# apache/orc

Hardware: AMD Instinct MI355X
Metric: decoded GB/s + Mvalues/s device-resident, RLEv2 int64 column at 1/2/4/8 GPU (higher is better)
Workload: dtype int64; 1 GPU; configs[1]: single int64 RLEv2-direct column, 10^8 rows, uncompressed stream resident in HBM, 1 MI355X per stripe; rows_per_gpu=100000000, encoding=RLEv2 DIRECT, W=64 (aligned), 512-value runs, signed (zigzag), stream_bytes=800390626, row_index_stride=10000, parallelism=stripe-sharded x1, kernel=rlev2_tiled_kernel, variant=0

## Files before the change

include/orcg_reader.h:

```cpp
#ifndef ORCG_READER_H
#define ORCG_READER_H

#include "orcg.h"

#ifdef __cplusplus
extern "C" {
#endif

enum {
  ORCG_TYPE_BOOLEAN = 0, ORCG_TYPE_BYTE = 1, ORCG_TYPE_SHORT = 2, ORCG_TYPE_INT = 3, ORCG_TYPE_LONG = 4,
  ORCG_TYPE_FLOAT = 5, ORCG_TYPE_DOUBLE = 6, ORCG_TYPE_STRING = 7, ORCG_TYPE_BINARY = 8,
  ORCG_TYPE_TIMESTAMP = 9, ORCG_TYPE_LIST = 10, ORCG_TYPE_MAP = 11, ORCG_TYPE_STRUCT = 12,
  ORCG_TYPE_UNION = 13, ORCG_TYPE_DECIMAL = 14, ORCG_TYPE_DATE = 15, ORCG_TYPE_VARCHAR = 16,
  ORCG_TYPE_CHAR = 17, ORCG_TYPE_TIMESTAMP_INSTANT = 18
};
enum { ORCG_COMPRESSION_NONE = 0, ORCG_COMPRESSION_ZLIB = 1, ORCG_COMPRESSION_SNAPPY = 2,
       ORCG_COMPRESSION_LZO = 3, ORCG_COMPRESSION_LZ4 = 4, ORCG_COMPRESSION_ZSTD = 5 };

typedef struct orcg_reader orcg_reader;

typedef struct {
  uint32_t kind;
  uint32_t num_subtypes;
  uint32_t maximum_length;
// ... 93 lines not shown
int orcg_reader_last_timings(const orcg_reader* r, double* out5);
int orcg_reader_last_stream_stats(const orcg_reader* r, uint64_t* out2);
typedef struct orcg_reader_metrics {
  uint64_t reader_call;
  uint64_t reader_inclusive_latency_us;
  uint64_t decompression_call;
  uint64_t decompression_latency_us;
  uint64_t decoding_call;
  uint64_t decoding_latency_us;
  uint64_t byte_decoding_call;
  uint64_t byte_decoding_latency_us;
  uint64_t io_count;
  uint64_t io_blocking_latency_us;
  uint64_t selected_row_group_count;
  uint64_t evaluated_row_group_count;
  uint64_t read_range_cache_hits;
  uint64_t read_range_cache_misses;
} orcg_reader_metrics;
int orcg_reader_get_metrics(orcg_reader* r, orcg_reader_metrics* out);
int orcg_reader_reset_metrics(orcg_reader* r);
int orcg_reader_set_metrics_timing(orcg_reader* r, int on);
uint64_t orcg_reader_last_batched_streams(const orcg_reader* r);
uint64_t orcg_reader_last_stage_bytes(const orcg_reader* r);
int orcg_reader_set_stream_batching(orcg_reader* r, int on);

#ifdef __cplusplus
}
#endif
#endif
```

orc_amd/_lib.py:

```python
import ctypes
import os

HERE = os.path.dirname(os.path.abspath(__file__))
LIB_PATH = os.path.join(HERE, os.environ.get("ORCG_LIB", "liborcgpu.so"))

ORCG_OK = 0
ORCG_PARSE_ERROR = 1
ORCG_INVALID_ARGUMENT = 2
ORCG_DEVICE_ERROR = 3
ORCG_OUT_OF_MEMORY = 4


class OrcError(RuntimeError):
    status = None


class ParseError(OrcError):

    status = ORCG_PARSE_ERROR


class InvalidArgument(OrcError):

    status = ORCG_INVALID_ARGUMENT
# ... 145 lines not shown
    ("orcg_reader_stripe_column", [vp, u64, u32, ctypes.POINTER(ColumnView)], i32),
    ("orcg_reader_copy_to_host", [vp, vp, vp, u64], i32),
    ("orcg_reader_last_timings", [vp, ctypes.POINTER(ctypes.c_double)], i32),
    ("orcg_reader_last_stream_stats", [vp, ctypes.POINTER(u64)], i32),
    ("orcg_reader_get_metrics", [vp, ctypes.POINTER(u64)], i32),
    ("orcg_reader_reset_metrics", [vp], i32),
    ("orcg_reader_set_metrics_timing", [vp, i32], i32),
    ("orcg_reader_content_length", [vp], u64),
    ("orcg_reader_software_version", [vp], cp),
    ("orcg_reader_num_metadata", [vp], u32),
    ("orcg_reader_metadata_key", [vp, u32], cp),
    ("orcg_reader_metadata_value", [vp, u32, ctypes.POINTER(u64)], vp),
    ("orcg_reader_set_lazy_dictionary", [vp, i32], i32),
    ("orcg_reader_set_hive11_decimal", [vp, i32, i32], i32),
    ("orcg_reader_hive11_scale", [vp], i32),
    ("orcg_reader_set_read_type", [vp, cp], i32),
    ("orcg_reader_set_throw_on_schema_evolution_overflow", [vp, i32], i32),
    ("orcg_reader_read_type", [vp, u32, ctypes.POINTER(TypeInfo)], i32),
    ("orcg_reader_set_zone_rules", [vp, cp, cp, u64], i32),
    ("orcg_reader_set_timezone_name", [vp, cp], i32),
    ("orcg_reader_set_local_timezone", [vp, cp], i32),
    ("orcg_reader_last_batched_streams", [vp], u64),
    ("orcg_reader_last_stage_bytes", [vp], u64),
    ("orcg_reader_set_stream_batching", [vp, i32], i32),
    ("orcg_reader_is_selected", [vp, u32], i32),
    ("orcg_row_reader_create", [vp, ctypes.POINTER(RowReaderOptions), ctypes.POINTER(vp)], i32),
    ("orcg_row_reader_destroy", [vp], None),
    ("orcg_row_reader_next", [vp, u64, ctypes.POINTER(u64)], i32),
    ("orcg_row_reader_is_selected", [vp, u32], i32),
    ("orcg_row_reader_stripe", [vp], u64),
    ("orcg_row_reader_row_number", [vp], u64),
    ("orcg_host_alloc", [u64], vp),
    ("orcg_host_free", [vp], None),
    ("orcg_row_reader_last_error", [vp], cp),
    ("orcg_row_reader_timings", [vp, ctypes.POINTER(ctypes.c_double)], i32),
    ("orcg_row_reader_seek_to_row", [vp, u64], i32),
    ("orcg_row_reader_column", [vp, u32, ctypes.POINTER(ColumnView), ctypes.POINTER(u64), ctypes.POINTER(u64)],
     i32),
]

i64 = ctypes.c_int64
SIGNATURES += [
    ("orcg_arrow_validity_device", [vp, vp, u64, vp, u64, ctypes.POINTER(u64)], i32),
    ("orcg_arrow_fixed_device", [vp, i32, vp, vp, u64, vp, u64], i32),
    ("orcg_arrow_offsets_device", [vp, vp, vp, vp, u64, vp, u64], i32),
    ("orcg_arrow_dict_strings_device", [vp, i32, vp, vp, u64, vp, u64, vp, u64, vp, u64, vp, u64,
# ... 71 lines not shown
```

orc_amd/build.py:

```python
import os
import subprocess
import sys

HERE = os.path.dirname(os.path.abspath(__file__))
CSRC = os.path.join(HERE, "csrc")
PROF = os.environ.get("ORCG_PHASE_PROF", "") == "1"
AB = os.environ.get("ORCG_AB", "") == "1"
OUT = os.path.join(HERE, "liborcgpu_prof.so" if PROF else ("liborcgpu_ab.so" if AB else "liborcgpu.so"))
OBJ = os.path.join(HERE, "build_prof" if PROF else ("build_ab" if AB else "build"))
ARCH = os.environ.get("ORCG_OFFLOAD_ARCH", "gfx950")

SOURCES = ["rlev2_kernels.hip", "rlev2_tiled.hip", "rlev2_expand.hip", "byterle_kernels.hip", "column_kernels.hip", "rlev1_kernels.hip", "decimal_kernels.hip", "convert_kernels.hip", "arrow_kernels.hip", "orcg_api.cpp", "multi_launch.cpp", "rlev1_api.cpp", "orc_file.cpp", "reader_api.cpp", "reader_prepare.cpp",
           "reader_collect.cpp", "reader_streams.cpp", "reader_decode.cpp", "reader_fork.cpp", "reader_stripes.cpp",
           "row_reader.cpp", "byterle_api.cpp", "decimal_api.cpp", "convert_api.cpp", "arrow_api.cpp", "arrow_export.cpp", "timezone.cpp", "encoder.cpp", "java_face.cpp"]
if PROF or AB:
    SOURCES.append("probe_kernels.hip")
HEADERS = ["orcg_internal.hh", "device_util.hh", "rlev2_device.hh", "orc_file.hh", "timezone.hh", "reader_layout.hh", "reader_internal.hh", "read_type.hh", "arrow_internal.hh", os.path.join("..", "..", "include", "orcg.h"),
           os.path.join("..", "..", "include", "orcg_reader.h"), os.path.join("..", "..", "include", "orcg_arrow.h")]

HIPCC = os.environ.get("HIPCC", "/opt/rocm/bin/hipcc")
FLAGS = ["-O3", "-std=c++17", "-fPIC", "-Wall", "-Wno-unused-function", "-Wno-unused-result", "-Wno-unused-value"]
if PROF:
    FLAGS.append("-DORCG_PHASE_PROF")
if PROF or AB:
    FLAGS.extend(os.environ.get("ORCG_AB_FLAGS", "").split())


def _mtime(p):
    return os.path.getmtime(p) if os.path.exists(p) else 0.0


def build(force=False, verbose=False):
    os.makedirs(OBJ, exist_ok=True)
    hdr_time = max(_mtime(os.path.join(CSRC, h)) for h in HEADERS)
    objs, cmds = [], []
    for s in SOURCES:
        src = os.path.join(CSRC, s)
        obj = os.path.join(OBJ, s + ".o")
        objs.append(obj)
        if not force and _mtime(obj) > max(_mtime(src), hdr_time):
# ... 30 lines not shown
```

orc_amd/csrc/orc_file.cpp:

```cpp
#include "orc_file.hh"

#include <dlfcn.h>
#include <string.h>
#include <zlib.h>


namespace orcg {
namespace file {
namespace {

struct Pb {
  const uint8_t* p;
  const uint8_t* end;
  bool ok = true;
  Pb(const uint8_t* b, uint64_t n) : p(b), end(b + n) {}
  bool more() const { return ok && p < end; }
  uint64_t varint() {
    uint64_t r = 0;
    for (int sh = 0; sh < 70; sh += 7) {
      if (p >= end) {
        ok = false;
        return 0;
      }
      const uint8_t b = *p++;
// ... 88 lines not shown
      uint32_t ef, ew;
      while (e.more() && e.key(ef, ew)) {
        if (ef == 1 && ew == 2) {
          Pb q = e.bytes();
          while (q.more()) pos.push_back(q.varint());
          if (!q.ok) return false;
        } else if (ef == 1 && ew == 0) {
          pos.push_back(e.varint());
        } else {
          e.skip(ew);
        }
      }
      if (!e.ok) return false;
      entries.push_back(std::move(pos));
    } else {
      m.skip(w);
    }
  }
  return m.ok;
}

namespace {

bool snappy_decompress(const uint8_t* in, uint64_t n, uint8_t* out, uint64_t cap, uint64_t& out_len,
                       std::string& err) {
  const uint8_t* p = in;
  const uint8_t* end = in + n;
  uint64_t ulen = 0;
  for (int sh = 0;; sh += 7) {
    if (p >= end || sh > 35) { err = "snappy: bad length"; return false; }
    const uint8_t b = *p++;
    ulen |= (uint64_t)(b & 0x7f) << sh;
    if (!(b & 0x80)) break;
  }
  if (ulen > cap) { err = "snappy: output exceeds the compression block size"; return false; }
  uint64_t o = 0;
  while (p < end) {
    const uint8_t tag = *p++;
    const uint32_t kind = tag & 3u;
    if (kind == 0) {
      uint64_t len = (tag >> 2) + 1u;
      if (len > 60) {
        const uint32_t nb = (uint32_t)len - 60;
        if ((uint64_t)(end - p) < nb) { err = "snappy: truncated literal"; return false; }
        len = 0;
        for (uint32_t i = 0; i < nb; ++i) len |= (uint64_t)p[i] << (8 * i);
        len += 1;
        p += nb;
      }
      if ((uint64_t)(end - p) < len || o + len > ulen) { err = "snappy: literal out of range"; return false; }
      memcpy(out + o, p, len);
      p += len;
      o += len;
    } else {
      uint64_t len, off;
      if (kind == 1) {
        if (p >= end) { err = "snappy: truncated copy"; return false; }
// ... 107 lines not shown
      if (dist == 0) {
        if (ip != ie) return fail("data after the end of the block");
        out_len = op;
        return true;
      }
      dist += 0x4000;
    }
    if (!copy_match(dist, len)) return fail("match outside the output");
    const uint64_t lit = ip[-2] & 3u;
    if (lit) {
      if (!literals(lit)) return fail("literal run past the end");
      state = 2;
    } else {
      state = 0;
    }
  }
}

}

typedef int (*lz4_fn)(const char*, char*, int, int);
typedef size_t (*zstd_fn)(void*, size_t, const void*, size_t);
typedef unsigned (*zstd_err_fn)(size_t);

struct DynCodecs {
  lz4_fn lz4 = nullptr;
  zstd_fn zstd = nullptr;
  zstd_err_fn zstd_is_error = nullptr;
  DynCodecs() {
    if (void* h = dlopen("liblz4.so.1", RTLD_NOW | RTLD_LOCAL)) lz4 = (lz4_fn)dlsym(h, "LZ4_decompress_safe");
    if (void* h = dlopen("libzstd.so.1", RTLD_NOW | RTLD_LOCAL)) {
      const zstd_fn d = (zstd_fn)dlsym(h, "ZSTD_decompress");
      const zstd_err_fn e = (zstd_err_fn)dlsym(h, "ZSTD_isError");
      if (d && e) {
        zstd = d;
        zstd_is_error = e;
      }
    }
  }
};

const DynCodecs& codecs() {
  static DynCodecs c;
  return c;
}

}

const char* compression_name(uint32_t c) {
  switch (c) {
    case kNone: return "none";
    case kZlib: return "zlib";
    case kSnappy: return "snappy";
    case kLzo: return "lzo";
    case kLz4: return "lz4";
    case kZstd: return "zstd";
  }
  return "unknown";
}
// ... 156 lines not shown
    case kLz4: {
      const auto& k = codecs();
      if (!k.lz4) { err = "lz4 codec library (liblz4.so.1) not available"; return false; }
      const int r = k.lz4((const char*)in, (char*)dst, (int)c.src_len, (int)cap);
      if (r < 0) { err = "Corrupt lz4 compressed block"; return false; }
      c.dst_len = (uint64_t)r;
      return true;
    }
    case kZstd: {
      const auto& k = codecs();
      if (!k.zstd) { err = "zstd codec library (libzstd.so.1) not available"; return false; }
      const size_t r = k.zstd(dst, cap, in, c.src_len);
      if (k.zstd_is_error(r)) { err = "Corrupt zstd compressed block"; return false; }
      c.dst_len = r;
      return true;
    }
    case kLzo:
      return lzo_decompress(in, c.src_len, dst, cap, c.dst_len, err);
  }
  err = "Unknown compression type";
  return false;
}

bool read_range(const uint8_t* file, uint64_t off, uint64_t len, uint32_t compression, uint64_t block_size,
                std::vector<uint8_t>& out, std::string& err) {
  std::vector<Chunk> chunks;
  if (!split_chunks(file, off, len, compression, chunks, err)) return false;
  out.clear();
  for (auto& c : chunks) {
    const uint64_t at = out.size();
    const uint64_t cap = c.original ? c.src_len : block_size;
    out.resize(at + cap);
    if (!decompress_chunk(compression, file, c, out.data() + at, cap, err)) return false;
    out.resize(at + c.dst_len);
  }
  return true;
}

}
}
```

orc_amd/csrc/orc_file.hh:

```
#pragma once

#include <stdint.h>

#include <string>
#include <vector>

namespace orcg {
namespace file {

enum Compression { kNone = 0, kZlib = 1, kSnappy = 2, kLzo = 3, kLz4 = 4, kZstd = 5 };

struct PostScript {
  uint64_t footer_length = 0;
  uint32_t compression = kNone;
  uint64_t block_size = 256 * 1024;
  std::vector<uint32_t> version;
  uint64_t metadata_length = 0;
  uint32_t writer_version = 0;
  std::string magic;
};

struct StripeInfo {
  uint64_t offset = 0, index_length = 0, data_length = 0, footer_length = 0, num_rows = 0;
};
// ... 40 lines not shown
};

struct StripeFooter {
  std::vector<StreamInfo> streams;
  std::vector<ColumnEncoding> encodings;
  std::string writer_timezone;
};

struct Chunk {
  uint64_t src_off = 0, src_len = 0;
  bool original = true;
  uint64_t dst_off = 0, dst_len = 0;
};

bool parse_postscript(const uint8_t* p, uint64_t n, PostScript& ps);
bool parse_footer(const uint8_t* p, uint64_t n, Footer& f);
bool parse_stripe_footer(const uint8_t* p, uint64_t n, uint64_t stripe_offset, StripeFooter& sf);
bool parse_row_index(const uint8_t* p, uint64_t n, std::vector<std::vector<uint64_t>>& entries);

bool split_chunks(const uint8_t* file, uint64_t off, uint64_t len, uint32_t compression, std::vector<Chunk>& out,
                  std::string& err);
bool decompress_chunk(uint32_t compression, const uint8_t* file, Chunk& c, uint8_t* dst, uint64_t cap,
                      std::string& err);
bool read_range(const uint8_t* file, uint64_t off, uint64_t len, uint32_t compression, uint64_t block_size,
                std::vector<uint8_t>& out, std::string& err);

const char* compression_name(uint32_t c);

}
}
```

orc_amd/csrc/reader_api.cpp:

```cpp
#include <fcntl.h>
#include <sys/mman.h>
#include <sys/stat.h>
#include <unistd.h>

#include "reader_internal.hh"

static thread_local std::string t_open_error;

orcg_reader::~orcg_reader() {
  if (ev_pre) (void)hipEventDestroy(ev_pre);
  if (h_pub) (void)hipHostFree(h_pub);
  slots.clear();
  if (mapped) munmap(mapped, file_len);
  if (h_sync) (void)hipHostFree(h_sync);
  for (Flight& f : flights) {
    if (f.h_defer) (void)hipHostFree(f.h_defer);
    if (f.h_rb) (void)hipHostFree(f.h_rb);
    for (const EvPair& p : f.ev_used) ev_pool.push_back(p.a), ev_pool.push_back(p.b);
    if (f.done) (void)hipEventDestroy(f.done);
    for (hipEvent_t e : {f.ev_up0, f.ev_up1, f.ev_dec})
      if (e) (void)hipEventDestroy(e);
  }
  for (hipEvent_t e : ev_pool) (void)hipEventDestroy(e);
}
// ... 357 lines not shown
int orcg_reader_get_metrics(orcg_reader* r, orcg_reader_metrics* out) {
  if (!r || !out) return ORCG_INVALID_ARGUMENT;
  std::lock_guard<std::mutex> lk(r->mu);
  static_assert(sizeof(orcg_reader_metrics) == 14 * sizeof(uint64_t), "orcg_reader_metrics layout");
  uint64_t* o = (uint64_t*)out;
  for (int i = 0; i < 14; ++i) o[i] = r->metrics[i].load(std::memory_order_relaxed);
  return ORCG_OK;
}

int orcg_reader_reset_metrics(orcg_reader* r) {
  if (!r) return ORCG_INVALID_ARGUMENT;
  std::lock_guard<std::mutex> lk(r->mu);
  for (auto& m : r->metrics) m.store(0, std::memory_order_relaxed);
  return ORCG_OK;
}

int orcg_reader_set_metrics_timing(orcg_reader* r, int on) {
  if (!r) return ORCG_INVALID_ARGUMENT;
  std::lock_guard<std::mutex> lk(r->mu);
  r->metrics_timing = on != 0;
  return ORCG_OK;
}
uint64_t orcg_reader_last_stage_bytes(const orcg_reader* r) { return r ? r->stage_bytes : 0; }

int orcg_reader_set_stream_batching(orcg_reader* r, int on) {
  if (!r) return ORCG_INVALID_ARGUMENT;
  r->batch_on = on != 0;
  return ORCG_OK;
}

}
```

orc_amd/csrc/reader_internal.hh:

```
#pragma once

#include <algorithm>
#include <atomic>
#include <cstdio>
#include <chrono>
#include <condition_variable>
#include <cstring>
#include <deque>
#include <functional>
#include <map>
#include <memory>
#include <mutex>
#include <thread>

#include "../../include/orcg_reader.h"
#include "orc_file.hh"
#include "orcg_internal.hh"
#include "read_type.hh"
#include "reader_layout.hh"
#include "timezone.hh"

namespace orcg {
namespace reader {

using namespace orcg::file;

inline double now_s() {
  return std::chrono::duration<double>(std::chrono::steady_clock::now().time_since_epoch()).count();
}

inline unsigned host_threads() {
  if (const char* e = getenv("ORCG_HOST_THREADS")) {
    const int v = atoi(e);
    if (v > 0) return (unsigned)v;
  }
  const unsigned hc = std::thread::hardware_concurrency();
  return std::max(1u, std::min(16u, hc ? hc : 1u));
}

template <typename F>
void parallel_for(size_t n, F&& f, uint64_t work_bytes = ~0ull, uint64_t bytes_per_thread = 1) {
  const uint64_t by_work = std::max<uint64_t>(1, work_bytes / std::max<uint64_t>(1, bytes_per_thread));
  const unsigned nt = (unsigned)std::min<uint64_t>(std::min<size_t>(host_threads(), n), by_work);
  if (nt <= 1) {
    for (size_t i = 0; i < n; ++i) f(i);
    return;
  }
  std::atomic<size_t> next{0};
  std::vector<std::thread> ts;
  for (unsigned t = 0; t < nt; ++t)
    ts.emplace_back([&] {
      for (size_t i; (i = next.fetch_add(1)) < n;) f(i);
    });
  for (auto& t : ts) t.join();
}

constexpr int64_t kOrcEpochUtc = tz::kOrcEpochUtc;

struct ZoneEntry {
  std::unique_ptr<tz::Zone> zone;
  std::string err;
  int64_t* d_tab = nullptr;
  uint32_t words = 0;
  ~ZoneEntry() {
    if (d_tab) (void)hipFree(d_tab);
  }
};

inline bool range_ok(uint64_t off, uint64_t len, uint64_t end) { return off <= end && len <= end - off; }

inline bool is_supported(const file::TypeInfo& t, const ZoneEntry* writer_zone) {
  const uint32_t k = t.kind;
  if (k == ORCG_TYPE_UNION) return true;
  if (k == ORCG_TYPE_DECIMAL) return true;
  if (k == ORCG_TYPE_TIMESTAMP) return writer_zone != nullptr;
  if (k == ORCG_TYPE_TIMESTAMP_INSTANT) return true;
  return k <= ORCG_TYPE_CHAR || k == ORCG_TYPE_DATE || k == ORCG_TYPE_VARCHAR;
// ... 82 lines not shown
  std::string text;
};

struct Col : ColView {
  bool supported = false;
  std::string stream_err;
  StreamBuf s[kNumSlots];
  bool nulls_deferred = false;
};

struct HostStage {
  uint64_t stripe = ~0ull;
  const ZoneEntry* writer_zone = nullptr;
  std::vector<Col> cols;
  uint8_t* h = nullptr;
  size_t cap = 0;
  uint64_t used = 0;
  int rc = ORCG_OK;
  std::string err;
  double t_parse = 0, t_decomp = 0, t_plan = 0;
  uint64_t ngroups = 0;
  uint64_t n_pos = 0, n_plan = 0;
  uint64_t n_chunks = 0;
  uint64_t n_io = 0;
  double t_io = 0;
  uint64_t io_sink = 0;
  uint64_t rows_off = 0;
  uint64_t slack = 0;
  ~HostStage() { pinned_free(h); }
  bool pinned_mapped = false;
  bool ensure(uint64_t bytes, uint64_t keep) {
    if (bytes <= cap) return true;
    const uint64_t ncap = std::max<uint64_t>(bytes + (bytes >> 2), 1 << 20) + slack;
    uint8_t* nh = (uint8_t*)pinned_alloc(ncap);
    if (!nh) return false;
    if (h) {
      if (keep) memcpy(nh, h, keep);
      pinned_free(h);
    }
    h = nh;
    cap = ncap;
    pinned_mapped = ncap < (size_t(8) << 20);
    return true;
  }
  int fail(int status, const std::string& m) {
    rc = status;
// ... 74 lines not shown
  rt::Tree file_tree() const;
  struct Active {
    orcg_reader* r;
    Active(orcg_reader* r_, Ctx* c, const std::vector<uint8_t>& sel, bool lazy, const ZoneEntry* rtz,
           const std::string& ltz, std::shared_ptr<const ReadPlan> rd, bool evo)
        : r(r_) {
      r->read = std::move(rd);
      r->evo_throw = evo;
      r->ctx = c;
      r->selected = sel;
      r->lazy_dict = lazy;
      r->reader_tz = rtz ? rtz : r->resolve_zone("GMT");
      r->local_tz = ltz;
    }
    ~Active() { r->ctx = nullptr; }
  };
  const uint8_t* file = nullptr;
  uint64_t file_len = 0;
  void* mapped = nullptr;
  PostScript ps;
  Footer footer;
  std::string last_error;
  HostStage stages[3];
  bool decimal_as_long = false;
  int32_t hive11_scale = 6;
  bool hive11_throw = true;
  std::string software_version;
  std::vector<std::unique_ptr<DevSlot>> slots;
  size_t nslots = 0;
  HostStage* H = nullptr;
  DevSlot* D = nullptr;
  double timings[5] = {0, 0, 0, 0, 0};
  uint64_t stream_stats[2] = {0, 0};
  enum {
    kMReaderCall, kMReaderLatency, kMDecompressCall, kMDecompressLatency, kMDecodeCall, kMDecodeLatency,
    kMByteCall, kMByteLatency, kMIOCount, kMIOLatency, kMSelectedRG, kMEvaluatedRG, kMCacheHits, kMCacheMisses
  };
  std::atomic<uint64_t> metrics[14] = {};
  void madd(int i, uint64_t v) { metrics[i].fetch_add(v, std::memory_order_relaxed); }
  bool metrics_timing = false;
  std::vector<hipEvent_t> ev_pool;
  hipEvent_t ev_get() {
    if (ev_pool.empty()) {
      hipEvent_t e = nullptr;
      if (hipEventCreate(&e) != hipSuccess) return nullptr;
      return e;
// ... 10 lines not shown
    const int rc = f();
    if (b) (void)hipEventRecord(b, ctx->stream);
    if (a && b) F->ev_used.push_back(EvPair{a, b, kind});
    else {
      if (a) ev_pool.push_back(a);
      if (b) ev_pool.push_back(b);
    }
    return rc;
  }
  void collect_event_times() {
    double us[2] = {0, 0};
    for (const EvPair& p : F->ev_used) {
      float ms = 0;
      if (hipEventElapsedTime(&ms, p.a, p.b) == hipSuccess) us[p.kind] += ms * 1e3;
      ev_pool.push_back(p.a);
      ev_pool.push_back(p.b);
    }
    F->ev_used.clear();
    madd(kMDecodeLatency, (uint64_t)us[0]);
    madd(kMByteLatency, (uint64_t)us[1]);
  }
  uint64_t batched_streams = 0;
  uint64_t stage_bytes = 0;

  struct Flight {
    HostStage* hs = nullptr;
    DevSlot* ds = nullptr;
    uint64_t* h_defer = nullptr;
    size_t defer_cap = 0, defer_used = 0;
    std::vector<std::pair<uint32_t, std::function<int()>>> checks;
    uint64_t* h_rb = nullptr;
    size_t h_rb_cap = 0, rb_words = 0, rb_used = 0;
    std::vector<EvPair> ev_used;
    hipEvent_t done = nullptr;
    hipEvent_t ev_up0 = nullptr, ev_up1 = nullptr, ev_dec = nullptr;
    bool ev_split = false;
    bool enqueued = false;
    int rc = ORCG_OK;
    uint32_t err_col = 0;
    std::string err_msg;
    double t0 = 0, t1 = 0;
  };
  Flight flights[2];
  Flight* F = &flights[0];
  static constexpr uint32_t kNoCol = 0xffffffffu;
  uint32_t cur_col = kNoCol, err_col = kNoCol;
// ... 197 lines not shown
```

orc_amd/csrc/reader_prepare.cpp:

```cpp
#include "reader_internal.hh"

int orcg_reader::open_tail() {
  if (file_len < 4) return fail(ORCG_PARSE_ERROR, "File size too small");
  const uint64_t ps_len = file[file_len - 1];
  if (ps_len < 3) return fail(ORCG_PARSE_ERROR, "Invalid ORC postscript length");
  if (memcmp(file + file_len - 1 - 3, "ORC", 3) != 0 && memcmp(file, "ORC", 3) != 0)
    return fail(ORCG_PARSE_ERROR, "Not an ORC file");
  if (file_len < 1 + ps_len)
    return fail(ORCG_PARSE_ERROR, "Invalid ORC postscript length: " + std::to_string(ps_len) +
                                      ", file length = " + std::to_string(file_len));
  if (!parse_postscript(file + file_len - 1 - ps_len, ps_len, ps))
    return fail(ORCG_PARSE_ERROR, "Failed to parse the postscript");
  if (ps.block_size == 0) ps.block_size = 256 * 1024;
  decimal_as_long = ps.version.size() == 2 && ps.version[0] == 1 && ps.version[1] == 9999;
  if (ps.footer_length >= file_len - 1 - ps_len)
    return fail(ORCG_PARSE_ERROR, "Invalid tail size: footerSize=" + std::to_string(ps.footer_length) +
                                      ", postscriptLength=" + std::to_string(ps_len) +
                                      ", fileLength=" + std::to_string(file_len));
  if (ps.compression > kZstd) return fail(ORCG_PARSE_ERROR, "Unknown compression type");
  std::vector<uint8_t> fbytes;
  std::string err;
  const uint64_t tail = 1 + ps_len + ps.footer_length;
  if (!read_range(file, file_len - tail, ps.footer_length, ps.compression, ps.block_size, fbytes, err))
    return fail(ORCG_PARSE_ERROR, err);
// ... 114 lines not shown
    Need nd{st.column, slot, {}, st.offset};
    if (!split_chunks(file, st.offset, st.length, ps.compression, nd.chunks, err)) {
      if (hs.cols[st.column].stream_err.empty()) hs.cols[st.column].stream_err = err;
      continue;
    }
    needs.push_back(std::move(nd));
  }
  return ORCG_OK;
}

int orcg_reader::load_streams(HostStage& hs, std::vector<Need>& needs, double* t_inflate, uint64_t* used) const {
  {
    const double ti = now_s();
    uint64_t sink = 0;
    for (const Need& nd : needs)
      for (const Chunk& ch : nd.chunks) {
        const uint8_t* b = file + ch.src_off;
        for (uint64_t o = 0; o < ch.src_len; o += 4096) sink += ((const volatile uint8_t*)b)[o];
      }
    hs.io_sink = sink;
    hs.t_io = now_s() - ti;
    hs.n_io = needs.size() + 1;
  }
  uint64_t at = 0;
  std::vector<std::pair<size_t, size_t>> all;
  for (size_t i = 0; i < needs.size(); ++i) {
    at = (at + 255) & ~(uint64_t)255;
    for (size_t j = 0; j < needs[i].chunks.size(); ++j) {
      Chunk& ch = needs[i].chunks[j];
      ch.dst_off = at;
      at += ch.original ? ch.src_len : ps.block_size;
      all.emplace_back(i, j);
    }
  }
  if (!hs.ensure(at + 64, 0)) return hs.fail(ORCG_OUT_OF_MEMORY, "pinned staging allocation failed");
  *t_inflate = now_s();
  std::vector<std::string> errs(all.size());
  std::atomic<bool> bad{false};
  uint64_t src_bytes = 0;
  for (auto& nd : needs)
    for (auto& ch : nd.chunks) src_bytes += ch.src_len;
  parallel_for(all.size(), [&](size_t q) {
    Chunk& ch = needs[all[q].first].chunks[all[q].second];
    const uint64_t cap = ch.original ? ch.src_len : ps.block_size;
    if (!decompress_chunk(ps.compression, file, ch, hs.h + ch.dst_off, cap, errs[q])) bad = true;
  }, src_bytes, ps.compression == kNone ? (1u << 20) : (64u << 10));
  if (bad)
    for (auto& e : errs)
      if (!e.empty()) return hs.fail(ORCG_PARSE_ERROR, e);
  uint64_t w = 0;
  for (size_t i = 0; i < needs.size(); ++i) {
    w = (w + 255) & ~(uint64_t)255;
    const uint64_t s0 = w;
    for (auto& ch : needs[i].chunks) {
      if (ch.dst_off != w) memmove(hs.h + w, hs.h + ch.dst_off, ch.dst_len);
      w += ch.dst_len;
    }
    StreamBuf& sb = hs.cols[needs[i].col].s[needs[i].slot];
    sb.present = true;
    sb.host_off = s0;
    sb.len = w - s0;
  }
  hs.n_chunks = all.size();
  *used = w;
  return ORCG_OK;
}

bool orcg_reader::column_positions(size_t col, Col& c, const StreamInfo& ri, uint64_t G, const std::vector<int>& need_of,
                                   const std::vector<Need>& needs) const {
  const bool compressed = ps.compression != kNone;
  std::vector<StreamDesc> order;
  for (const StreamDesc& d : layout((uint32_t)col, c))
    if (d.positioned()) order.push_back(d);
  bool ok = !order.empty();
  for (auto& o : order) ok = ok && c.s[o.slot].present && need_of[col * kNumSlots + o.slot] >= 0;
  if (!ok) return false;
  std::vector<uint8_t> ib;
  std::vector<std::vector<uint64_t>> entries;
  std::string e2;
  if (!read_range(file, ri.offset, ri.length, ps.compression, ps.block_size, ib, e2) ||
      !parse_row_index(ib.data(), ib.size(), entries) || entries.size() != G)
    return false;
  std::vector<std::vector<std::pair<uint64_t, uint64_t>>> cmap(order.size());
  for (size_t o = 0; o < order.size(); ++o) {
    const Need& nd = needs[need_of[col * kNumSlots + order[o].slot]];
// ... 54 lines not shown
    sb.pos = true;
    sb.trip = std::move(trips[o]);
  }
  return true;
}

void orcg_reader::map_row_index(uint64_t s, const StripeFooter& sf, const std::vector<int>& row_index,
                                const std::vector<Need>& needs, HostStage& hs) const {
  const StripeInfo& si = footer.stripes[s];
  const size_t nt = footer.types.size();
  hs.ngroups = 0;
  const char* no_ri = getenv("ORCG_NO_ROW_INDEX");
  if (footer.row_index_stride == 0 || si.num_rows == 0 || (no_ri && no_ri[0] == '1')) return;
  const uint64_t G = (si.num_rows + footer.row_index_stride - 1) / footer.row_index_stride;
  std::vector<int> need_of(nt * kNumSlots, -1);
  for (size_t i = 0; i < needs.size(); ++i) need_of[needs[i].col * kNumSlots + needs[i].slot] = (int)i;
  std::atomic<bool> any{false};
  uint64_t ri_bytes = 0;
  for (size_t col = 0; col < nt; ++col)
    if (row_index[col] >= 0) ri_bytes += sf.streams[row_index[col]].length;
  parallel_for(nt, [&](size_t col) {
    if (row_index[col] < 0) return;
    if (column_positions(col, hs.cols[col], sf.streams[row_index[col]], G, need_of, needs)) any = true;
  }, ri_bytes, 16u << 10);
  if (any) hs.ngroups = G;
}

void orcg_reader::build_plans(const std::vector<uint8_t>& selected, HostStage& hs, std::vector<StreamBuf*>& rle) const {
  const size_t nt = footer.types.size();
  std::vector<uint8_t> alone(nt, 0);
  for (size_t i = 0; i < nt; ++i) {
    const Col& c = hs.cols[i];
    const bool down = alone[i] || c.s[kSlotPresent].present || c.kind == ORCG_TYPE_LIST || c.kind == ORCG_TYPE_MAP;
    if (c.s[kSlotPresent].present) alone[i] = 1;
    if (down)
      for (uint32_t st : footer.types[i].subtypes)
        if (st < nt && st > i) alone[st] = 1;
  }
  std::vector<int> rle_kind;
  for (size_t i = 0; i < nt; ++i) {
    Col& c = hs.cols[i];
    if (!selected[i] || !c.supported) continue;
    const StreamLayout lay = layout((uint32_t)i, c);
    for (int sl : {kSlotPresent, kSlotData, kSlotLength, kSlotSecondary}) {
      StreamBuf& sb = c.s[sl];
      if (!sb.present) continue;
      const StreamDesc* d = lay.find(sl);
// ... 8 lines not shown
        } else if (kind == 2 && alone[i] && per_group > (8u << 10) && long_runs(hs.h + sb.host_off, sb.len)) {
          fine = true;
        } else {
          continue;
        }
        sb.pos = false;
        sb.trip.clear();
      }
      rle.push_back(&sb);
      rle_kind.push_back(fine ? 3 : kind);
    }
  }
  uint64_t plan_bytes = 0;
  for (auto* sb : rle) plan_bytes += sb->len;
  parallel_for(rle.size(), [&](size_t q) {
    StreamBuf& sb = *rle[q];
    const uint8_t* p = hs.h + sb.host_off;
    constexpr uint32_t byte_seg = 4u << 10;
    if (rle_kind[q] == 0) sb.plan.reset(make_byte_plan(p, sb.len, byte_seg, byte_seg));
    else if (rle_kind[q] == 1)
      sb.plan.reset(make_v1_plan(p, sb.len, sb.len <= kV1SmallStream ? (1u << 10) : (16u << 10), 8192));
    else if (rle_kind[q] == 3) sb.plan.reset(make_plan(p, sb.len, 8u << 10, 4096));
    else sb.plan.reset(make_plan(p, sb.len, 16u << 10, 8192));
  }, plan_bytes, 512u << 10);
  hs.n_plan = rle.size();
}

int orcg_reader::layout_staging(uint64_t s, HostStage& hs, const std::vector<StreamBuf*>& rle, uint64_t w) const {
  const StripeInfo& si = footer.stripes[s];
  const size_t nt = footer.types.size();
  hs.n_pos = 0;
  for (auto& c : hs.cols)
    for (auto& sb : c.s) hs.n_pos += sb.pos ? 1 : 0;
  hs.slack = upload_tail_bytes(nt, v1_segments(hs), (si.num_rows + 2047) / 2048 + 1);
  uint64_t seg_bytes = 0;
  for (auto* sb : rle) seg_bytes += ((sb->plan->segs.size() * sizeof(orcg_segment)) + 255) & ~(uint64_t)255;
  w = (w + 255) & ~(uint64_t)255;
  if (!hs.ensure(w + seg_bytes + 64, w)) return hs.fail(ORCG_OUT_OF_MEMORY, "pinned staging allocation failed");
  for (auto* sb : rle) {
    sb->seg_off = w;
    const size_t nb = sb->plan->segs.size() * sizeof(orcg_segment);
    if (nb) memcpy(hs.h + w, sb->plan->segs.data(), nb);
    w = (w + nb + 255) & ~(uint64_t)255;
  }
  uint64_t rg_bytes = hs.ngroups ? ((hs.ngroups * 8 + 255) & ~(uint64_t)255) : 0;
  for (auto& c : hs.cols)
    for (auto& sb : c.s)
// ... 44 lines not shown
```

orc_amd/csrc/reader_stripes.cpp:

```cpp
#include "reader_internal.hh"

int orcg_reader::poll_counts(const std::vector<CountSrc>& srcs, uint64_t* out) {
  if (!h_pub) {
    void* h = nullptr;
    if (hipHostMalloc(&h, kPubSlots * kPubStride * 8, hipHostMallocCoherent | hipHostMallocMapped) != hipSuccess) {
      (void)hipGetLastError();
      return 1;
    }
    void* d = nullptr;
    if (hipHostGetDevicePointer(&d, h, 0) != hipSuccess) {
      (void)hipGetLastError();
      (void)hipHostFree(h);
      return 1;
    }
    memset(h, 0, kPubSlots * kPubStride * 8);
    h_pub = (uint64_t*)h;
    d_pub = (uint64_t*)d;
  }
  std::vector<Ctx*> order;
  std::vector<PublishArgs> args;
  std::vector<std::vector<size_t>> where;
  for (size_t i = 0; i < srcs.size(); ++i) {
    size_t g = 0;
    while (g < order.size() && order[g] != srcs[i].lane) ++g;
// ... 292 lines not shown
  madd(kMDecompressCall, hs.n_chunks);
  madd(kMDecompressLatency, (uint64_t)(hs.t_decomp * 1e6));
  madd(kMIOCount, hs.n_io);
  madd(kMIOLatency, (uint64_t)(hs.t_io * 1e6));
  if (metrics_timing) collect_event_times();
  else madd(kMDecodeLatency, (uint64_t)((t_end - fl.t1) * 1e6));
  return rc;
}

int orcg_reader::upload_and_decode(HostStage& hs, DevSlot& ds) {
  issue(hs, ds, flights[0]);
  return finish(flights[0]);
}

int orcg_reader::read_stripes(uint64_t first, uint64_t count) {
  if (!ctx) return fail(ORCG_INVALID_ARGUMENT, "reader has no device context");
  if (first > footer.stripes.size() || count > footer.stripes.size() - first)
    return fail(ORCG_INVALID_ARGUMENT, "stripe index out of range");
  hipSetDevice(ctx->device);
  for (auto& t : timings) t = 0;
  stream_stats[0] = stream_stats[1] = 0;
  batched_streams = 0;
  stage_bytes = 0;
  while (slots.size() < count) slots.emplace_back(new DevSlot());
  nslots = 0;
  if (count == 0) return ORCG_OK;
  std::mutex pm;
  std::condition_variable pcv;
  uint64_t prepared = 0, released = 0;
  bool quit = false;
  std::thread prep([&] {
    for (uint64_t k = 0; k < count; ++k) {
      {
        std::unique_lock<std::mutex> lk(pm);
        pcv.wait(lk, [&] { return quit || k < released + 3; });
        if (quit) return;
      }
      prepare(first + k, stages[k % 3]);
      {
        std::lock_guard<std::mutex> lk(pm);
        prepared = k + 1;
      }
      pcv.notify_all();
      if (stages[k % 3].rc) return;
    }
  });
  auto release = [&](uint64_t n) {
    {
      std::lock_guard<std::mutex> lk(pm);
      released = n;
    }
    pcv.notify_all();
  };
  int rc = ORCG_OK;
  bool pending = false;
  for (uint64_t k = 0; k <= count; ++k) {
    bool issued = false;
    if (k < count) {
      {
        std::unique_lock<std::mutex> lk(pm);
        pcv.wait(lk, [&] { return prepared > k; });
      }
      HostStage& cur = stages[k % 3];
      timings[0] += cur.t_parse;
      timings[1] += cur.t_decomp;
      timings[2] += cur.t_plan;
      stream_stats[0] += cur.n_pos;
      stream_stats[1] += cur.n_plan;
      if (cur.rc) {
        if (pending) {
          const int prc = finish(flights[(k - 1) & 1]);
          if (!prc) nslots = k;
          rc = prc ? prc : fail(cur.rc, cur.err);
        } else {
          rc = fail(cur.rc, cur.err);
        }
        pending = false;
        break;
      }
      issue(cur, *slots[k], flights[k & 1]);
      issued = true;
    }
    if (pending) {
      const int prc = finish(flights[(k - 1) & 1]);
      release(k);
      if (prc) {
        rc = prc;
        if (issued) {
          (void)hipEventSynchronize(flights[k & 1].done);
          issued = false;
        }
// ... 15 lines not shown
```

orc_amd/reader.py:

```python
import ctypes
import datetime
import decimal

import numpy as np

from . import _lib
from ._lib import check
from .rle import Context, default_context

BOOLEAN, BYTE, SHORT, INT, LONG, FLOAT, DOUBLE, STRING, BINARY, TIMESTAMP, LIST, MAP, STRUCT, UNION, \
    DECIMAL, DATE, VARCHAR, CHAR, TIMESTAMP_INSTANT = range(19)
KIND_NAMES = ["boolean", "tinyint", "smallint", "int", "bigint", "float", "double", "string", "binary",
              "timestamp", "array", "map", "struct", "uniontype", "decimal", "date", "varchar", "char",
              "timestamp with local time zone"]
COMPRESSION_NAMES = ["NONE", "ZLIB", "SNAPPY", "LZO", "LZ4", "ZSTD"]
SUPPORTED = {BOOLEAN, BYTE, SHORT, INT, LONG, FLOAT, DOUBLE, STRING, BINARY, LIST, MAP, STRUCT, DATE, VARCHAR,
             CHAR, UNION}
STRING_KINDS = (STRING, VARCHAR, CHAR, BINARY)
_EPOCH = datetime.date(1970, 1, 1)
_DECIMAL_CTX = decimal.Context(prec=40)


_KEEP = object()

# ... 382 lines not shown
    def set_local_timezone(self, name):
        check(self._L.orcg_reader_set_local_timezone(self._h, None if name is None else name.encode()), self._err)

    def set_lazy_dictionary(self, on=True):
        check(self._L.orcg_reader_set_lazy_dictionary(self._h, int(bool(on))), self._err)

    def create_row_reader(self, include=None, offset=0, length=None, lazy_dictionary=False, tight_numeric=False,
                          timezone=None, read_type=_KEEP, throw_on_overflow=_KEEP):
        return RowReader(self, include=include, offset=offset, length=length, lazy_dictionary=lazy_dictionary,
                         tight_numeric=tight_numeric, timezone=timezone, read_type=read_type,
                         throw_on_overflow=throw_on_overflow)

    def last_timings(self):
        t = (ctypes.c_double * 5)()
        check(self._L.orcg_reader_last_timings(self._h, t))
        return {"host_parse_s": t[0], "host_decompress_s": t[1], "host_plan_s": t[2], "h2d_s": t[3],
                "device_decode_s": t[4]}

    def last_stream_stats(self):
        t = (ctypes.c_uint64 * 2)()
        check(self._L.orcg_reader_last_stream_stats(self._h, t))
        return {"row_index": t[0], "host_plan": t[1],
                "batched": int(self._L.orcg_reader_last_batched_streams(self._h)),
                "stage_bytes": int(self._L.orcg_reader_last_stage_bytes(self._h))}

    METRIC_NAMES = ("ReaderCall", "ReaderInclusiveLatencyUs", "DecompressionCall", "DecompressionLatencyUs",
                    "DecodingCall", "DecodingLatencyUs", "ByteDecodingCall", "ByteDecodingLatencyUs", "IOCount",
                    "IOBlockingLatencyUs", "SelectedRowGroupCount", "EvaluatedRowGroupCount",
                    "ReadRangeCacheHits", "ReadRangeCacheMisses")

    def metrics(self, reset=False):
        t = (ctypes.c_uint64 * len(self.METRIC_NAMES))()
        check(self._L.orcg_reader_get_metrics(self._h, t))
        if reset:
            check(self._L.orcg_reader_reset_metrics(self._h))
        return dict(zip(self.METRIC_NAMES, (int(x) for x in t)))

    def set_metrics_timing(self, on=True):
        check(self._L.orcg_reader_set_metrics_timing(self._h, int(bool(on))), self._err)

    def set_stream_batching(self, on=True):
        check(self._L.orcg_reader_set_stream_batching(self._h, int(bool(on))), self._err)


    def arrow_schema(self, dictionary=False):
        import pyarrow as pa

# ... 194 lines not shown
```

Before: 3017 GB/s.

## Size decompression slots from codec headers and reuse a persistent host worker pool

```diff
diff --git a/include/orcg_reader.h b/include/orcg_reader.h
--- a/include/orcg_reader.h
+++ b/include/orcg_reader.h
@@ -139,6 +139,7 @@
 int orcg_reader_set_metrics_timing(orcg_reader* r, int on);
 uint64_t orcg_reader_last_batched_streams(const orcg_reader* r);
 uint64_t orcg_reader_last_stage_bytes(const orcg_reader* r);
+uint64_t orcg_reader_last_moved_bytes(const orcg_reader* r);
 int orcg_reader_set_stream_batching(orcg_reader* r, int on);
 
 #ifdef __cplusplus
diff --git a/orc_amd/_lib.py b/orc_amd/_lib.py
--- a/orc_amd/_lib.py
+++ b/orc_amd/_lib.py
@@ -191,6 +191,7 @@
     ("orcg_reader_set_local_timezone", [vp, cp], i32),
     ("orcg_reader_last_batched_streams", [vp], u64),
     ("orcg_reader_last_stage_bytes", [vp], u64),
+    ("orcg_reader_last_moved_bytes", [vp], u64),
     ("orcg_reader_set_stream_batching", [vp, i32], i32),
     ("orcg_reader_is_selected", [vp, u32], i32),
     ("orcg_row_reader_create", [vp, ctypes.POINTER(RowReaderOptions), ctypes.POINTER(vp)], i32),
diff --git a/orc_amd/build.py b/orc_amd/build.py
--- a/orc_amd/build.py
+++ b/orc_amd/build.py
@@ -15,7 +15,7 @@
            "row_reader.cpp", "byterle_api.cpp", "decimal_api.cpp", "convert_api.cpp", "arrow_api.cpp", "arrow_export.cpp", "timezone.cpp", "encoder.cpp", "java_face.cpp"]
 if PROF or AB:
     SOURCES.append("probe_kernels.hip")
-HEADERS = ["orcg_internal.hh", "device_util.hh", "rlev2_device.hh", "orc_file.hh", "timezone.hh", "reader_layout.hh", "reader_internal.hh", "read_type.hh", "arrow_internal.hh", os.path.join("..", "..", "include", "orcg.h"),
+HEADERS = ["orcg_internal.hh", "device_util.hh", "rlev2_device.hh", "orc_file.hh", "chunk_placement.hh", "host_workers.hh", "timezone.hh", "reader_layout.hh", "reader_internal.hh", "read_type.hh", "arrow_internal.hh", os.path.join("..", "..", "include", "orcg.h"),
            os.path.join("..", "..", "include", "orcg_reader.h"), os.path.join("..", "..", "include", "orcg_arrow.h")]
 
 HIPCC = os.environ.get("HIPCC", "/opt/rocm/bin/hipcc")
diff --git a/orc_amd/csrc/chunk_placement.hh b/orc_amd/csrc/chunk_placement.hh
--- /dev/null
+++ b/orc_amd/csrc/chunk_placement.hh
@@ -0,0 +1,111 @@
+#pragma once
+
+#include <string.h>
+
+#include <algorithm>
+#include <string>
+#include <vector>
+
+#include "orc_file.hh"
+
+namespace orcg {
+namespace reader {
+
+inline uint64_t slot_bytes(const file::Chunk& c, uint64_t hint, uint64_t block_size) {
+  if (c.original) return c.src_len;
+  return std::min(hint, block_size);
+}
+
+struct ChunkSlots {
+  std::vector<size_t> first;
+  std::vector<uint64_t> slot;
+  std::vector<uint64_t> off;
+  uint64_t total = 0;
+  size_t streams() const { return first.empty() ? 0 : first.size() - 1; }
+};
+
+inline void place_chunks(ChunkSlots& p) {
+  p.off.resize(p.slot.size());
+  uint64_t at = 0;
+  for (size_t i = 0; i < p.streams(); ++i) {
+    at = (at + 255) & ~(uint64_t)255;
+    for (size_t q = p.first[i]; q < p.first[i + 1]; ++q) {
+      p.off[q] = at;
+      at += p.slot[q];
+    }
+  }
+  p.total = at;
+}
+
+struct ChunkMove {
+  uint64_t dst, src, len;
+};
+
+struct ChunkRepair {
+  bool ok = true;
+  std::vector<ChunkMove> moves;
+  std::vector<uint64_t> stream_off, stream_len;
+  uint64_t used = 0;
+  uint64_t moved = 0;
+  bool packed = false;
+};
+
+inline ChunkRepair repair_chunks(const ChunkSlots& p, const std::vector<uint64_t>& actual) {
+  ChunkRepair r;
+  const size_t ns = p.streams();
+  uint64_t bytes = 0, tight = 0;
+  for (size_t i = 0; i < ns; ++i) {
+    tight = (tight + 255) & ~(uint64_t)255;
+    for (size_t q = p.first[i]; q < p.first[i + 1]; ++q) {
+      if (actual[q] > p.slot[q]) {
+        r.ok = false;
+        return r;
+      }
+      tight += actual[q];
+      bytes += actual[q];
+    }
+  }
+  uint64_t kept_end = 0;
+  if (ns) {
+    kept_end = p.first[ns - 1] < p.first[ns] ? p.off[p.first[ns - 1]] : p.total;
+    for (size_t q = p.first[ns - 1]; q < p.first[ns]; ++q) kept_end += actual[q];
+  }
+  r.packed = kept_end - tight > bytes / 16;
+  uint64_t w = 0;
+  for (size_t i = 0; i < ns; ++i) {
+    const size_t q0 = p.first[i], q1 = p.first[i + 1];
+    w = (w + 255) & ~(uint64_t)255;
+    if (!r.packed && q0 < q1) w = p.off[q0];
+    r.stream_off.push_back(w);
+    for (size_t q = q0; q < q1; ++q) {
+      if (p.off[q] != w && actual[q]) {
+        r.moves.push_back(ChunkMove{w, p.off[q], actual[q]});
+        r.moved += actual[q];
+      }
+      w += actual[q];
+    }
+    r.stream_len.push_back(w - r.stream_off.back());
+  }
+  r.used = w;
+  return r;
+}
+
+inline void apply_moves(uint8_t* base, const ChunkRepair& r) {
+  for (const ChunkMove& m : r.moves) memmove(base + m.dst, base + m.src, m.len);
+}
+
+inline bool inflate_into_slot(uint32_t compression, const uint8_t* file, file::Chunk& c, uint8_t* dst, uint64_t slot,
+                              uint64_t block_size, std::string& err, bool* outgrew) {
+  *outgrew = false;
+  if (file::decompress_chunk(compression, file, c, dst, slot, err)) return true;
+  if (c.original || slot >= block_size) return false;
+  std::vector<uint8_t> scratch(block_size);
+  err.clear();
+  if (!file::decompress_chunk(compression, file, c, scratch.data(), block_size, err)) return false;
+  if (c.dst_len > slot) *outgrew = true;
+  else if (c.dst_len) memcpy(dst, scratch.data(), c.dst_len);
+  return true;
+}
+
+}
+}
diff --git a/orc_amd/csrc/host_workers.hh b/orc_amd/csrc/host_workers.hh
--- /dev/null
+++ b/orc_amd/csrc/host_workers.hh
@@ -0,0 +1,108 @@
+#pragma once
+
+#include <stdint.h>
+#include <stdlib.h>
+
+#include <algorithm>
+#include <atomic>
+#include <condition_variable>
+#include <functional>
+#include <mutex>
+#include <thread>
+#include <vector>
+
+namespace orcg {
+namespace reader {
+
+inline unsigned host_threads() {
+  if (const char* e = getenv("ORCG_HOST_THREADS")) {
+    const int v = atoi(e);
+    if (v > 0) return (unsigned)v;
+  }
+  const unsigned hc = std::thread::hardware_concurrency();
+  return std::max(1u, std::min(16u, hc ? hc : 1u));
+}
+
+class HostWorkers {
+ public:
+  ~HostWorkers() {
+    {
+      std::lock_guard<std::mutex> lk(mu_);
+      quit_ = true;
+    }
+    wake_.notify_all();
+    for (auto& t : ts_) t.join();
+  }
+  bool run(unsigned helpers, const std::function<void()>& body) {
+    std::unique_lock<std::mutex> job(job_mu_, std::try_to_lock);
+    if (!job.owns_lock()) return false;
+    {
+      std::lock_guard<std::mutex> lk(mu_);
+      while (ts_.size() < helpers) {
+        const unsigned idx = (unsigned)ts_.size();
+        const uint64_t seen = gen_;
+        ts_.emplace_back([this, idx, seen] { loop(idx, seen); });
+      }
+      body_ = &body;
+      take_ = pending_ = helpers;
+      ++gen_;
+    }
+    wake_.notify_all();
+    body();
+    std::unique_lock<std::mutex> lk(mu_);
+    done_.wait(lk, [&] { return pending_ == 0; });
+    body_ = nullptr;
+    return true;
+  }
+
+ private:
+  void loop(unsigned idx, uint64_t seen) {
+    std::unique_lock<std::mutex> lk(mu_);
+    for (;;) {
+      wake_.wait(lk, [&] { return quit_ || gen_ != seen; });
+      if (quit_) return;
+      seen = gen_;
+      if (idx >= take_) continue;
+      const std::function<void()>* body = body_;
+      lk.unlock();
+      (*body)();
+      lk.lock();
+      if (--pending_ == 0) done_.notify_one();
+    }
+  }
+  std::mutex job_mu_;
+  std::mutex mu_;
+  std::condition_variable wake_, done_;
+  std::vector<std::thread> ts_;
+  const std::function<void()>* body_ = nullptr;
+  uint64_t gen_ = 0;
+  unsigned take_ = 0, pending_ = 0;
+  bool quit_ = false;
+};
+
+inline bool host_pool_on() {
+  const char* e = getenv("ORCG_HOST_POOL");
+  return !(e && e[0] == '0');
+}
+
+template <typename F>
+void parallel_for(size_t n, F&& f, uint64_t work_bytes = ~0ull, uint64_t bytes_per_thread = 1,
+                  HostWorkers* pool = nullptr) {
+  const uint64_t by_work = std::max<uint64_t>(1, work_bytes / std::max<uint64_t>(1, bytes_per_thread));
+  const unsigned nt = (unsigned)std::min<uint64_t>(std::min<size_t>(host_threads(), n), by_work);
+  if (nt <= 1) {
+    for (size_t i = 0; i < n; ++i) f(i);
+    return;
+  }
+  std::atomic<size_t> next{0};
+  const std::function<void()> body = [&] {
+    for (size_t i; (i = next.fetch_add(1)) < n;) f(i);
+  };
+  if (pool && host_pool_on() && pool->run(nt - 1, body)) return;
+  std::vector<std::thread> ts;
+  for (unsigned t = 0; t < nt; ++t) ts.emplace_back(body);
+  for (auto& t : ts) t.join();
+}
+
+}
+}
diff --git a/orc_amd/csrc/orc_file.cpp b/orc_amd/csrc/orc_file.cpp
--- a/orc_amd/csrc/orc_file.cpp
+++ b/orc_amd/csrc/orc_file.cpp
@@ -134,17 +134,22 @@
 
 namespace {
 
+bool snappy_length(const uint8_t*& p, const uint8_t* end, uint64_t& ulen) {
+  ulen = 0;
+  for (int sh = 0;; sh += 7) {
+    if (p >= end || sh > 35) return false;
+    const uint8_t b = *p++;
+    ulen |= (uint64_t)(b & 0x7f) << sh;
+    if (!(b & 0x80)) return true;
+  }
+}
+
 bool snappy_decompress(const uint8_t* in, uint64_t n, uint8_t* out, uint64_t cap, uint64_t& out_len,
                        std::string& err) {
   const uint8_t* p = in;
   const uint8_t* end = in + n;
   uint64_t ulen = 0;
-  for (int sh = 0;; sh += 7) {
-    if (p >= end || sh > 35) { err = "snappy: bad length"; return false; }
-    const uint8_t b = *p++;
-    ulen |= (uint64_t)(b & 0x7f) << sh;
-    if (!(b & 0x80)) break;
-  }
+  if (!snappy_length(p, end, ulen)) { err = "snappy: bad length"; return false; }
   if (ulen > cap) { err = "snappy: output exceeds the compression block size"; return false; }
   uint64_t o = 0;
   while (p < end) {
@@ -298,11 +303,15 @@
 typedef int (*lz4_fn)(const char*, char*, int, int);
 typedef size_t (*zstd_fn)(void*, size_t, const void*, size_t);
 typedef unsigned (*zstd_err_fn)(size_t);
+typedef unsigned long long (*zstd_content_fn)(const void*, size_t);
+typedef size_t (*zstd_frame_fn)(const void*, size_t);
 
 struct DynCodecs {
   lz4_fn lz4 = nullptr;
   zstd_fn zstd = nullptr;
   zstd_err_fn zstd_is_error = nullptr;
+  zstd_content_fn zstd_content_size = nullptr;
+  zstd_frame_fn zstd_frame_size = nullptr;
   DynCodecs() {
     if (void* h = dlopen("liblz4.so.1", RTLD_NOW | RTLD_LOCAL)) lz4 = (lz4_fn)dlsym(h, "LZ4_decompress_safe");
     if (void* h = dlopen("libzstd.so.1", RTLD_NOW | RTLD_LOCAL)) {
@@ -311,6 +320,12 @@
       if (d && e) {
         zstd = d;
         zstd_is_error = e;
+        const zstd_content_fn cs = (zstd_content_fn)dlsym(h, "ZSTD_getFrameContentSize");
+        const zstd_frame_fn fs = (zstd_frame_fn)dlsym(h, "ZSTD_findFrameCompressedSize");
+        if (cs && fs) {
+          zstd_content_size = cs;
+          zstd_frame_size = fs;
+        }
       }
     }
   }
@@ -513,6 +528,26 @@
   return false;
 }
 
+uint64_t chunk_size_hint(uint32_t compression, const uint8_t* file, const Chunk& c) {
+  const uint8_t* in = file + c.src_off;
+  if (c.original) return c.src_len;
+  if (compression == kSnappy) {
+    const uint8_t* p = in;
+    uint64_t ulen = 0;
+    return snappy_length(p, in + c.src_len, ulen) ? ulen : kNoSizeHint;
+  }
+  if (compression == kZstd) {
+    const auto& k = codecs();
+    if (!k.zstd_content_size) return kNoSizeHint;
+    const unsigned long long n = k.zstd_content_size(in, c.src_len);
+    if (n >= ~0ull - 1) return kNoSizeHint;
+    const size_t fs = k.zstd_frame_size(in, c.src_len);
+    if (k.zstd_is_error(fs) || fs != c.src_len) return kNoSizeHint;
+    return n;
+  }
+  return kNoSizeHint;
+}
+
 bool read_range(const uint8_t* file, uint64_t off, uint64_t len, uint32_t compression, uint64_t block_size,
                 std::vector<uint8_t>& out, std::string& err) {
   std::vector<Chunk> chunks;
diff --git a/orc_amd/csrc/orc_file.hh b/orc_amd/csrc/orc_file.hh
--- a/orc_amd/csrc/orc_file.hh
+++ b/orc_amd/csrc/orc_file.hh
@@ -86,6 +86,8 @@
                   std::string& err);
 bool decompress_chunk(uint32_t compression, const uint8_t* file, Chunk& c, uint8_t* dst, uint64_t cap,
                       std::string& err);
+constexpr uint64_t kNoSizeHint = ~0ull;
+uint64_t chunk_size_hint(uint32_t compression, const uint8_t* file, const Chunk& c);
 bool read_range(const uint8_t* file, uint64_t off, uint64_t len, uint32_t compression, uint64_t block_size,
                 std::vector<uint8_t>& out, std::string& err);
 
diff --git a/orc_amd/csrc/reader_api.cpp b/orc_amd/csrc/reader_api.cpp
--- a/orc_amd/csrc/reader_api.cpp
+++ b/orc_amd/csrc/reader_api.cpp
@@ -403,6 +403,7 @@
   return ORCG_OK;
 }
 uint64_t orcg_reader_last_stage_bytes(const orcg_reader* r) { return r ? r->stage_bytes : 0; }
+uint64_t orcg_reader_last_moved_bytes(const orcg_reader* r) { return r ? r->moved_bytes : 0; }
 
 int orcg_reader_set_stream_batching(orcg_reader* r, int on) {
   if (!r) return ORCG_INVALID_ARGUMENT;
diff --git a/orc_amd/csrc/reader_internal.hh b/orc_amd/csrc/reader_internal.hh
--- a/orc_amd/csrc/reader_internal.hh
+++ b/orc_amd/csrc/reader_internal.hh
@@ -14,6 +14,8 @@
 #include <thread>
 
 #include "../../include/orcg_reader.h"
+#include "chunk_placement.hh"
+#include "host_workers.hh"
 #include "orc_file.hh"
 #include "orcg_internal.hh"
 #include "read_type.hh"
@@ -27,32 +29,6 @@
 
 inline double now_s() {
   return std::chrono::duration<double>(std::chrono::steady_clock::now().time_since_epoch()).count();
-}
-
-inline unsigned host_threads() {
-  if (const char* e = getenv("ORCG_HOST_THREADS")) {
-    const int v = atoi(e);
-    if (v > 0) return (unsigned)v;
-  }
-  const unsigned hc = std::thread::hardware_concurrency();
-  return std::max(1u, std::min(16u, hc ? hc : 1u));
-}
-
-template <typename F>
-void parallel_for(size_t n, F&& f, uint64_t work_bytes = ~0ull, uint64_t bytes_per_thread = 1) {
-  const uint64_t by_work = std::max<uint64_t>(1, work_bytes / std::max<uint64_t>(1, bytes_per_thread));
-  const unsigned nt = (unsigned)std::min<uint64_t>(std::min<size_t>(host_threads(), n), by_work);
-  if (nt <= 1) {
-    for (size_t i = 0; i < n; ++i) f(i);
-    return;
-  }
-  std::atomic<size_t> next{0};
-  std::vector<std::thread> ts;
-  for (unsigned t = 0; t < nt; ++t)
-    ts.emplace_back([&] {
-      for (size_t i; (i = next.fetch_add(1)) < n;) f(i);
-    });
-  for (auto& t : ts) t.join();
 }
 
 constexpr int64_t kOrcEpochUtc = tz::kOrcEpochUtc;
@@ -181,6 +157,7 @@
   uint64_t ngroups = 0;
   uint64_t n_pos = 0, n_plan = 0;
   uint64_t n_chunks = 0;
+  uint64_t moved_bytes = 0;
   uint64_t n_io = 0;
   double t_io = 0;
   uint64_t io_sink = 0;
@@ -301,6 +278,7 @@
   Footer footer;
   std::string last_error;
   HostStage stages[3];
+  mutable HostWorkers workers;
   bool decimal_as_long = false;
   int32_t hive11_scale = 6;
   bool hive11_throw = true;
@@ -357,6 +335,7 @@
   }
   uint64_t batched_streams = 0;
   uint64_t stage_bytes = 0;
+  uint64_t moved_bytes = 0;
 
   struct Flight {
     HostStage* hs = nullptr;
diff --git a/orc_amd/csrc/reader_prepare.cpp b/orc_amd/csrc/reader_prepare.cpp
--- a/orc_amd/csrc/reader_prepare.cpp
+++ b/orc_amd/csrc/reader_prepare.cpp
@@ -160,45 +160,63 @@
     hs.t_io = now_s() - ti;
     hs.n_io = needs.size() + 1;
   }
-  uint64_t at = 0;
   std::vector<std::pair<size_t, size_t>> all;
+  ChunkSlots place;
+  uint64_t src_bytes = 0;
   for (size_t i = 0; i < needs.size(); ++i) {
-    at = (at + 255) & ~(uint64_t)255;
+    place.first.push_back(all.size());
     for (size_t j = 0; j < needs[i].chunks.size(); ++j) {
-      Chunk& ch = needs[i].chunks[j];
+      const Chunk& ch = needs[i].chunks[j];
+      place.slot.push_back(slot_bytes(ch, chunk_size_hint(ps.compression, file, ch), ps.block_size));
+      all.emplace_back(i, j);
+      src_bytes += ch.src_len;
+    }
+  }
+  place.first.push_back(all.size());
+  *t_inflate = now_s();
+  ChunkRepair fix;
+  std::vector<uint64_t> actual(all.size());
+  for (;;) {
+    place_chunks(place);
+    if (!hs.ensure(place.total + 64, 0)) return hs.fail(ORCG_OUT_OF_MEMORY, "pinned staging allocation failed");
+    std::vector<std::string> errs(all.size());
+    std::atomic<bool> bad{false}, regrow{false};
+    parallel_for(all.size(), [&](size_t q) {
+      Chunk& ch = needs[all[q].first].chunks[all[q].second];
+      ch.dst_off = place.off[q];
+      bool outgrew = false;
+      if (!inflate_into_slot(ps.compression, file, ch, hs.h + ch.dst_off, place.slot[q], ps.block_size, errs[q],
+                             &outgrew))
+        bad = true;
+      if (outgrew) regrow = true;
+      actual[q] = ch.dst_len;
+    }, src_bytes, ps.compression == kNone ? (1u << 20) : (64u << 10), &workers);
+    if (bad)
+      for (auto& e : errs)
+        if (!e.empty()) return hs.fail(ORCG_PARSE_ERROR, e);
+    if (!regrow) {
+      fix = repair_chunks(place, actual);
+      break;
+    }
+    for (size_t q = 0; q < all.size(); ++q) {
+      const Chunk& ch = needs[all[q].first].chunks[all[q].second];
+      place.slot[q] = slot_bytes(ch, kNoSizeHint, ps.block_size);
+    }
+  }
+  apply_moves(hs.h, fix);
+  for (size_t i = 0; i < needs.size(); ++i) {
+    uint64_t at = fix.stream_off[i];
+    for (auto& ch : needs[i].chunks) {
       ch.dst_off = at;
-      at += ch.original ? ch.src_len : ps.block_size;
-      all.emplace_back(i, j);
-    }
-  }
-  if (!hs.ensure(at + 64, 0)) return hs.fail(ORCG_OUT_OF_MEMORY, "pinned staging allocation failed");
-  *t_inflate = now_s();
-  std::vector<std::string> errs(all.size());
-  std::atomic<bool> bad{false};
-  uint64_t src_bytes = 0;
-  for (auto& nd : needs)
-    for (auto& ch : nd.chunks) src_bytes += ch.src_len;
-  parallel_for(all.size(), [&](size_t q) {
-    Chunk& ch = needs[all[q].first].chunks[all[q].second];
-    const uint64_t cap = ch.original ? ch.src_len : ps.block_size;
-    if (!decompress_chunk(ps.compression, file, ch, hs.h + ch.dst_off, cap, errs[q])) bad = true;
-  }, src_bytes, ps.compression == kNone ? (1u << 20) : (64u << 10));
-  if (bad)
-    for (auto& e : errs)
-      if (!e.empty()) return hs.fail(ORCG_PARSE_ERROR, e);
-  uint64_t w = 0;
-  for (size_t i = 0; i < needs.size(); ++i) {
-    w = (w + 255) & ~(uint64_t)255;
-    const uint64_t s0 = w;
-    for (auto& ch : needs[i].chunks) {
-      if (ch.dst_off != w) memmove(hs.h + w, hs.h + ch.dst_off, ch.dst_len);
-      w += ch.dst_len;
+      at += ch.dst_len;
     }
     StreamBuf& sb = hs.cols[needs[i].col].s[needs[i].slot];
     sb.present = true;
-    sb.host_off = s0;
-    sb.len = w - s0;
-  }
+    sb.host_off = fix.stream_off[i];
+    sb.len = fix.stream_len[i];
+  }
+  const uint64_t w = fix.used;
+  hs.moved_bytes = fix.moved;
   hs.n_chunks = all.size();
   *used = w;
   return ORCG_OK;
@@ -299,7 +317,7 @@
   parallel_for(nt, [&](size_t col) {
     if (row_index[col] < 0) return;
     if (column_positions(col, hs.cols[col], sf.streams[row_index[col]], G, need_of, needs)) any = true;
-  }, ri_bytes, 16u << 10);
+  }, ri_bytes, 16u << 10, &workers);
   if (any) hs.ngroups = G;
 }
 
@@ -354,7 +372,7 @@
       sb.plan.reset(make_v1_plan(p, sb.len, sb.len <= kV1SmallStream ? (1u << 10) : (16u << 10), 8192));
     else if (rle_kind[q] == 3) sb.plan.reset(make_plan(p, sb.len, 8u << 10, 4096));
     else sb.plan.reset(make_plan(p, sb.len, 16u << 10, 8192));
-  }, plan_bytes, 512u << 10);
+  }, plan_bytes, 512u << 10, &workers);
   hs.n_plan = rle.size();
 }
 
diff --git a/orc_amd/csrc/reader_stripes.cpp b/orc_amd/csrc/reader_stripes.cpp
--- a/orc_amd/csrc/reader_stripes.cpp
+++ b/orc_amd/csrc/reader_stripes.cpp
@@ -338,6 +338,7 @@
   stream_stats[0] = stream_stats[1] = 0;
   batched_streams = 0;
   stage_bytes = 0;
+  moved_bytes = 0;
   while (slots.size() < count) slots.emplace_back(new DevSlot());
   nslots = 0;
   if (count == 0) return ORCG_OK;
@@ -383,6 +384,7 @@
       timings[2] += cur.t_plan;
       stream_stats[0] += cur.n_pos;
       stream_stats[1] += cur.n_plan;
+      moved_bytes += cur.moved_bytes;
       if (cur.rc) {
         if (pending) {
           const int prc = finish(flights[(k - 1) & 1]);
diff --git a/orc_amd/reader.py b/orc_amd/reader.py
--- a/orc_amd/reader.py
+++ b/orc_amd/reader.py
@@ -428,7 +428,8 @@
         check(self._L.orcg_reader_last_stream_stats(self._h, t))
         return {"row_index": t[0], "host_plan": t[1],
                 "batched": int(self._L.orcg_reader_last_batched_streams(self._h)),
-                "stage_bytes": int(self._L.orcg_reader_last_stage_bytes(self._h))}
+                "stage_bytes": int(self._L.orcg_reader_last_stage_bytes(self._h)),
+                "moved_bytes": int(self._L.orcg_reader_last_moved_bytes(self._h))}
 
     METRIC_NAMES = ("ReaderCall", "ReaderInclusiveLatencyUs", "DecompressionCall", "DecompressionLatencyUs",
                     "DecodingCall", "DecodingLatencyUs", "ByteDecodingCall", "ByteDecodingLatencyUs", "IOCount",
```

Measured after the change: 2985 GB/s (median of 4 runs). About the same (-1.0%).
